# yangliu9527/Object_SLAM

Hardware: AMD Instinct MI355X
Metric: frames/sec tracking+localBA (higher is better)
Workload: dtype f64

## Files before the change

object_slam_amd/csrc/lba.hip:

```cpp
#include <hip/hip_runtime.h>
#include <string.h>
#include <type_traits>
#include <stdint.h>

#include <algorithm>
#include <atomic>
#include <chrono>
#include <condition_variable>
#include <mutex>
#include <array>
#include <vector>

#include "common.h"
#include "se3_math.h"
#include "lane_ops.h"
#include "slam_pool.h"

namespace oslam {

#ifdef OSLAM_LBA_PROFILE
#define LBA_STAMP(i) do { if (tid == 0) { long long t_ = clock64(); prof[i] += t_ - tlast; tlast = t_; } } while (0)
#else
#define LBA_STAMP(i) do { } while (0)
#endif
// ... 2035 lines not shown
        else for (int i = 0; i < 16; i++) pr.poses_out[a * 16 + i] = pr.poses[a * 16 + i];
    }
    if (gid < pr.P * 3) pr.points_out[gid] = early ? pr.points[gid] : (float)X[gid];
    if (gid == 0) { pr.stats[0] = ct->its[0]; pr.stats[1] = ct->trials[0]; pr.stats[2] = ct->its[1]; pr.stats[3] = ct->trials[1]; }
}

#include "lba_win.inc"

}

using namespace oslam;


struct oslam_lba {
    int device = 0, max_batch = 0, max_kf = 0;
    DeviceBuffer in_d, work_d, out_d;
    PinnedBuffer in_h; size_t in_off = 0;
    PinnedBuffer out_h;
    PinnedBuffer h_ctrl;
    hipStream_t strm = nullptr;
    bool owns_strm = true;
    std::mutex* launch_gate = nullptr;
    bool device_pairs = true;
    long long prof_pre_upload_ns = 0;
    int wide = 1;
    size_t win_lds_max = 0;
    int edge_rec = 1;
    int schur_vinv = 1;
    int schur_tiles = 0;
    int chol_mode = 0;
    struct Prep {
        LbaProblem pr;
        const float* p_poses = nullptr; const uint8_t* p_fixed = nullptr; const float* p_points = nullptr;
        std::vector<int> ekf, ept, pt_start, pose_start, pose_edges, pstart, chunk_kf, chunk_e0, chunk_n, kf_chunk0, pt_edge, tile_p0, tile_s0, stg_edge;
        std::vector<int> thr_own, blk_thr, blk_slots;
        int TE = 0, TP = 0, region_doubles = 0, ngroup = 1, hs_global = 0;
        std::vector<float> eobs, einfo;
        std::vector<int2> pairs;
        size_t o_poses, o_fixed, o_points, o_ekf, o_ept, o_eobs, o_einfo, o_ptstart, o_posestart, o_poseedges, o_pairs, o_pstart;
        size_t o_chunk_kf, o_chunk_e0, o_chunk_n, o_kf_chunk0, o_pt_edge, o_tile_p0, o_tile_s0, o_stg_edge, o_thr_own, o_blk_thr, o_blk_slots;
        size_t o_out_poses, o_out_points, o_out_erase, o_out_stats;
        int nfree = 0, nblk = 1; size_t npairs = 0; bool dev_pairs = false;
        int layout = 0;
        std::vector<int> order;
    };
    std::vector<Prep> prep;
    int n_prep = 0;
    PinnedBuffer h_stop;
    int* d_stop = nullptr;
    size_t lds = 0;
    hipEvent_t ev0 = nullptr, ev1 = nullptr;
    int timing = 0;
    double kern_ms = 0;
    long long kern_launches = 0;
};

static void lba_time_begin(oslam_lba* h) { if (h->timing && h->ev0) (void)hipEventRecord(h->ev0, h->strm); }
static void lba_time_end(oslam_lba* h) { if (h->timing && h->ev1) (void)hipEventRecord(h->ev1, h->strm); }
static void lba_time_collect(oslam_lba* h, long long launches) {
    if (!h->timing || !h->ev0 || !h->ev1) return;
    float ms = 0.f;
    if (hipEventElapsedTime(&ms, h->ev0, h->ev1) == hipSuccess) { h->kern_ms += ms; h->kern_launches += launches; }
}

static int arena_reserve(DeviceBuffer& q, size_t bytes) {
    if (bytes > q.cap()) OSLAM_HIP_CHECK(hipDeviceSynchronize());
    return q.grow(bytes, 1u << 20);
}

static int in_take(oslam_lba* h, size_t bytes, size_t* off) {
    const size_t need = h->in_off + ((bytes + 255) & ~(size_t)255);
    if (need > h->in_h.cap()) {
        PinnedBuffer nb;
        OSLAM_HIP_CHECK(hipStreamSynchronize(h->strm));
        OSLAM_CHECK(nb.alloc(need + need / 2 + (1u << 20)));
        if (h->in_h.ptr()) memcpy(nb.ptr(), h->in_h.ptr(), h->in_off);
        h->in_h = std::move(nb);
    }
    *off = h->in_off;
    h->in_off = need;
    return OSLAM_OK;
}
static int in_put(oslam_lba* h, const void* src, size_t bytes, size_t* off) {
    const int rc = in_take(h, bytes, off);
    if (rc) return rc;
    if (bytes) memcpy(h->in_h.bytes() + *off, src, bytes);
    return OSLAM_OK;
}

extern "C" {

int oslam_lba_kernel_time(oslam_lba_t* h, int enable, double* ms_out, long long* launches_out) {
    if (!h) { set_error("NULL handle"); return OSLAM_E_INVALID; }
    OSLAM_HIP_CHECK(hipSetDevice(h->device));
    if (enable && !h->ev0) { OSLAM_HIP_CHECK(hipEventCreate(&h->ev0)); OSLAM_HIP_CHECK(hipEventCreate(&h->ev1)); }
    if (ms_out) *ms_out = h->kern_ms;
    if (launches_out) *launches_out = h->kern_launches;
    h->kern_ms = 0; h->kern_launches = 0;
    h->timing = enable;
    return OSLAM_OK;
}

static double* s_lba_trace_buf = nullptr;
static int s_lba_trace_cap = 0;
int oslam_lba_trace(oslam_lba_t* h, int cap) {
    if (!h || cap < 0) { set_error("oslam_lba_trace: bad argument"); return OSLAM_E_INVALID; }
    OSLAM_HIP_CHECK(hipSetDevice(h->device));
    OSLAM_HIP_CHECK(hipDeviceSynchronize());
    double* none = nullptr; int zero = 0;
    OSLAM_HIP_CHECK(hipMemcpyToSymbol(HIP_SYMBOL(g_lba_trace), &none, sizeof(none)));
    OSLAM_HIP_CHECK(hipMemcpyToSymbol(HIP_SYMBOL(g_lba_trace_cap), &zero, sizeof(zero)));
    if (s_lba_trace_buf) (void)hipFree(s_lba_trace_buf);
    s_lba_trace_buf = nullptr; s_lba_trace_cap = 0;
    if (cap == 0) return OSLAM_OK;
    OSLAM_HIP_CHECK(hipMalloc((void**)&s_lba_trace_buf, sizeof(double) * (1 + 6 * (size_t)cap)));
    OSLAM_HIP_CHECK(hipMemset(s_lba_trace_buf, 0, sizeof(double) * (1 + 6 * (size_t)cap)));
    s_lba_trace_cap = cap;
    OSLAM_HIP_CHECK(hipMemcpyToSymbol(HIP_SYMBOL(g_lba_trace), &s_lba_trace_buf, sizeof(s_lba_trace_buf)));
    OSLAM_HIP_CHECK(hipMemcpyToSymbol(HIP_SYMBOL(g_lba_trace_cap), &cap, sizeof(cap)));
// ... 75 lines not shown
    memcpy(out, h->out_h.bytes() + h->prep[0].o_out_stats, 64);
    return OSLAM_OK;
}

int oslam_lba_set_mode(oslam_lba_t* h, int wide) {
    if (!h || wide < 0 || wide > 2) { set_error("oslam_lba_set_mode: mode must be 0 (compact), 1 (wide) or 2 (one workgroup per window, LDS-resident)"); return OSLAM_E_INVALID; }
    h->wide = wide;
    return OSLAM_OK;
}

int oslam_lba_set_schur(oslam_lba_t* h, int mode) {
    if (!h || mode < 0 || mode > 3) { set_error("oslam_lba_set_schur: mode must be 0 (pair gather), 1 (LDS tiles), 2 (per call) or 3 (pair gather, host-built lists)"); return OSLAM_E_INVALID; }
    h->schur_tiles = mode == 3 ? 0 : mode;
    h->device_pairs = mode != 3 && !getenv("OSLAM_LBA_HOST_PAIRS");
    return OSLAM_OK;
}

int oslam_lba_set_solver(oslam_lba_t* h, int mode) {
    if (!h || mode < 0 || mode > 4) { set_error("oslam_lba_set_solver: bad argument"); return OSLAM_E_INVALID; }
    h->chol_mode = mode;
    return OSLAM_OK;
}

volatile int32_t* oslam_lba_stop_flag(oslam_lba_t* h) { return h ? h->h_stop.as<volatile int32_t>() : nullptr; }

}

static int lba_build_tiles(oslam_lba::Prep& q, const std::vector<int>& blk, int nfree, int nP, int nE, size_t region_bytes, char* err, size_t errn) {
#pragma clang diagnostic push
#pragma clang diagnostic ignored "-Wformat-security"
    auto fail = [&](int rc, const char* fmt, auto... a) { snprintf(err, errn, fmt, a...); return rc; };
#pragma clang diagnostic pop
    const std::vector<int>& pt_start = q.pt_start;
    const std::vector<int>& ekf = q.ekf;
    const int nblk = q.nblk;
    auto tof = [&](int x, int y) { return x * nfree - x * (x - 1) / 2 + (y - x); };
    int TP = kWinTilePointsMax, TE = kWinTileEdgesMax;
    while (TE > 128 && win_tile_doubles(TE, TP) * 8 > region_bytes) TE -= 32;
    q.TE = TE; q.TP = TP;
    q.tile_p0.clear(); q.tile_s0.clear(); q.stg_edge.clear();
    std::vector<long long> load(nblk, 0);
    {
        int np = 0, ns = 0;
        q.tile_p0.push_back(0); q.tile_s0.push_back(0);
        std::vector<int> fb;
        for (int p = 0; p < nP; p++) {
            fb.clear();
            for (int i = pt_start[p]; i < pt_start[p + 1]; i++) { const int b2 = blk[ekf[q.pt_edge[i]]]; if (b2 >= 0) fb.push_back(b2); }
            const int fe = (int)fb.size();
            if (np > 0 && (np + 1 > TP || ns + fe > TE)) { q.tile_p0.push_back(p); q.tile_s0.push_back((int)q.stg_edge.size()); np = 0; ns = 0; }
            for (int i = pt_start[p]; i < pt_start[p + 1]; i++) {
                const int e = q.pt_edge[i];
                if (blk[ekf[e]] >= 0) { q.stg_edge.push_back(e); ns++; }
            }
            for (int i = 0; i < fe; i++)
                for (int j = i; j < fe; j++) load[tof(fb[i], fb[j])]++;
            np++;
        }
        q.tile_p0.push_back(nP); q.tile_s0.push_back((int)q.stg_edge.size());
    }
    q.npairs = 0;
    for (int b2 = 0; b2 < nblk; b2++) q.npairs += (size_t)load[b2];
    {
        std::vector<int> cnt(nblk, 0);
        int used = 0;
        for (int b2 = 0; b2 < nblk; b2++) if (load[b2] > 0) { cnt[b2] = 1; used++; }
        const int G = std::max(1, (used + kWinThreads - 1) / kWinThreads);
// ... 22 lines not shown
        for (size_t i = 0; i < ord.size(); i++) {
            const int b2 = ord[i].second / 64, s2 = ord[i].second % 64, g = (int)(i % G), slot = g * kWinThreads + fill[g]++;
            q.thr_own[slot] = b2 | (s2 << 16) | (cnt[b2] << 24);
            slot_of[i] = slot;
        }
        std::vector<std::vector<int>> per(nblk);
        for (size_t i = 0; i < ord.size(); i++) { const int b2 = ord[i].second / 64, s2 = ord[i].second % 64; if ((int)per[b2].size() < cnt[b2]) per[b2].resize(cnt[b2]); per[b2][s2] = slot_of[i]; }
        for (int b2 = 0; b2 < nblk; b2++) {
            q.blk_thr[b2] = (int)q.blk_slots.size() | (cnt[b2] << 16);
            for (int s2 = 0; s2 < cnt[b2]; s2++) q.blk_slots.push_back(per[b2][s2]);
        }
        if (q.blk_slots.empty()) q.blk_slots.push_back(0);
    }
    return OSLAM_OK;
}

static int lba_build(const oslam_lba_t* h, oslam_lba::Prep& q, int layout, bool want_pairs, bool use_tiles, int nKF, const float* poses, const uint8_t* fixed, int nP, const float* points,
                     int nE, const int32_t* edge_kf, const int32_t* edge_pt, const float* edge_obs, const float* edge_invSigma2, const float K5[5], int use_stop_flag,
                     const float* poses_out, const float* points_out, const uint8_t* erase, int iters0, int iters1, int nstages, int robust0, float delta_mono,
                     float delta_stereo, char* err, size_t errn) {
#pragma clang diagnostic push
#pragma clang diagnostic ignored "-Wformat-security"
    auto fail = [&](int rc, const char* fmt, auto... a) { snprintf(err, errn, fmt, a...); return rc; };
#pragma clang diagnostic pop
    if (!h || !poses || !fixed || !points || !K5 || !poses_out || !points_out || (nE > 0 && (!edge_kf || !edge_pt || !edge_obs || !edge_invSigma2 || !erase)))
        return fail(OSLAM_E_INVALID, "NULL argument");
    if (nKF < 1 || nKF > h->max_kf || nP < 0 || nE < 0)
        return fail(OSLAM_E_CAPACITY, "problem (%d keyframes, %d points, %d edges) exceeds the handle capacity (%d keyframes per window)", nKF, nP, nE, h->max_kf);
    q.layout = layout;
    q.p_poses = poses; q.p_fixed = fixed; q.p_points = points;
    std::vector<int>& pt_start = q.pt_start; std::vector<int>& pose_start = q.pose_start;
    pt_start.assign(nP + 1, 0); pose_start.assign(nKF + 1, 0);
    std::vector<int>& order = q.order;
    order.resize(nE);
    for (int i = 0; i < nE; i++) {
        if (edge_kf[i] < 0 || edge_kf[i] >= nKF || edge_pt[i] < 0 || edge_pt[i] >= nP) return fail(OSLAM_E_INVALID, "edge %d references vertex out of range", i);
        pt_start[edge_pt[i] + 1]++;
        pose_start[edge_kf[i] + 1]++;
    }
    for (int p = 0; p < nP; p++) pt_start[p + 1] += pt_start[p];
    for (int k = 0; k < nKF; k++) pose_start[k + 1] += pose_start[k];
    {
        std::vector<int> cur(pt_start.begin(), pt_start.end() - 1);
        for (int i = 0; i < nE; i++) order[cur[edge_pt[i]]++] = i;
    }
    if (layout == 1) {
        std::vector<int> cur(pose_start.begin(), pose_start.end() - 1), o2(nE);
        for (int i = 0; i < nE; i++) o2[cur[edge_kf[order[i]]]++] = order[i];
        order.swap(o2);
    }
    std::vector<int>& ekf = q.ekf; std::vector<int>& ept = q.ept;
    ekf.resize(nE); ept.resize(nE); q.eobs.resize((size_t)nE * 3); q.einfo.resize(nE);
    for (int i = 0; i < nE; i++) {
        const int sidx = order[i];
        ekf[i] = edge_kf[sidx]; ept[i] = edge_pt[sidx]; q.einfo[i] = edge_invSigma2[sidx];
        for (int k = 0; k < 3; k++) q.eobs[(size_t)i * 3 + k] = edge_obs[(size_t)sidx * 3 + k];
    }
    int nfree = 0;
    for (int k = 0; k < nKF; k++) nfree += fixed[k] ? 0 : 1;
    if (nfree > kLbaMaxKF) return fail(OSLAM_E_CAPACITY, "%d free keyframes > %d", nfree, kLbaMaxKF);
    if (h->wide == 0 && nKF > kLbaMaxKF) return fail(OSLAM_E_CAPACITY, "%d keyframes > %d (compact layout; use mode 1 or 2)", nKF, kLbaMaxKF);
    q.nfree = nfree; q.nblk = std::max(1, nfree * (nfree + 1) / 2);
    std::vector<int> blk(nKF);
    for (int k = 0, nb = 0; k < nKF; k++) blk[k] = fixed[k] ? -1 : nb++;
    auto tof = [&](int x, int y) { return x * nfree - x * (x - 1) / 2 + (y - x); };
    q.npairs = 0; q.pairs.clear(); q.pstart.clear(); q.dev_pairs = false;
    if (layout == 0) {
        q.pose_edges.resize(nE);
        std::vector<int> cur(pose_start.begin(), pose_start.end() - 1);
        for (int i = 0; i < nE; i++) q.pose_edges[cur[ekf[i]]++] = i;
        std::vector<int> seen(nKF, -1);
        for (int p = 0; p < nP; p++)
            for (int i = pt_start[p]; i < pt_start[p + 1]; i++) {
                if (seen[ekf[i]] == p) return fail(OSLAM_E_INVALID, "duplicate observation of point %d in keyframe %d", p, ekf[i]);
                seen[ekf[i]] = p;
            }
        q.tile_p0.clear();
        if (want_pairs && use_tiles) {
            q.pt_edge.resize(nE);
            for (int i = 0; i < nE; i++) q.pt_edge[i] = i;
            for (int p = 0; p < nP; p++) std::sort(q.pt_edge.begin() + pt_start[p], q.pt_edge.begin() + pt_start[p + 1], [&](int x, int y) { return ekf[x] < ekf[y]; });
            const int rc = lba_build_tiles(q, blk, nfree, nP, nE, (size_t)kWinLdsMax, err, errn);
            if (rc) return rc;
        } else if (want_pairs && h->device_pairs && h->wide == 1) {
            size_t tot = 0;
            for (int p = 0; p < nP; p++) {
                if (pt_start[p + 1] - pt_start[p] > 65534) return fail(OSLAM_E_CAPACITY, "point %d has more than 65534 observations", p);
                size_t kf_ = 0;
                for (int i = pt_start[p]; i < pt_start[p + 1]; i++) kf_ += blk[ekf[i]] >= 0;
                tot += kf_ * (kf_ + 1) / 2;
            }
            q.npairs = tot; q.dev_pairs = true;
        } else if (want_pairs) {
            const int nblk = q.nblk;
            std::vector<int>& pstart = q.pstart;
            pstart.assign(nblk + 1, 0);
            for (int p = 0; p < nP; p++)
                for (int i = pt_start[p]; i < pt_start[p + 1]; i++) {
                    const int bi = blk[ekf[i]];
                    if (bi < 0) continue;
                    for (int j = pt_start[p]; j < pt_start[p + 1]; j++) {
                        const int bj = blk[ekf[j]];
                        if (bj >= bi) pstart[tof(bi, bj) + 1]++;
// ... 14 lines not shown
                }
        }
    } else {
        q.pt_edge.resize(nE);
        {
            std::vector<int> cur(pt_start.begin(), pt_start.end() - 1);
            for (int i = 0; i < nE; i++) q.pt_edge[cur[ept[i]]++] = i;
        }
        for (int p = 0; p < nP; p++)
            for (int i = pt_start[p] + 1; i < pt_start[p + 1]; i++)
                if (ekf[q.pt_edge[i]] == ekf[q.pt_edge[i - 1]]) return fail(OSLAM_E_INVALID, "duplicate observation of point %d in keyframe %d", p, ekf[q.pt_edge[i]]);
        q.chunk_kf.clear(); q.chunk_e0.clear(); q.chunk_n.clear(); q.kf_chunk0.assign(nKF + 1, 0);
        for (int k = 0; k < nKF; k++) {
            q.kf_chunk0[k] = (int)q.chunk_kf.size();
            for (int e0 = pose_start[k]; e0 < pose_start[k + 1]; e0 += 64) { q.chunk_kf.push_back(k); q.chunk_e0.push_back(e0); q.chunk_n.push_back(std::min(64, pose_start[k + 1] - e0)); }
        }
        q.kf_chunk0[nKF] = (int)q.chunk_kf.size();
        const size_t region_bytes = h->win_lds_max - win_persist_bytes(nKF, nfree);
        size_t hs_d = (size_t)win_hs_doubles(nfree);
        q.hs_global = hs_d * 8 > region_bytes ? 1 : 0;
        if (q.hs_global) { const size_t n6 = 6 * (size_t)nfree, pw = ((n6 + 1 + kMB - 1) / kMB + 1) * kMB; hs_d = (size_t)kMB * pw + n6 + 2 * kMB; }
        { const int rc = lba_build_tiles(q, blk, nfree, nP, nE, region_bytes, err, errn); if (rc) return rc; }
        q.region_doubles = (int)std::max(hs_d, win_tile_doubles(q.TE, q.TP));
    }
    LbaProblem& pr = q.pr;
    memset(&pr, 0, sizeof(pr));
    pr.K = nKF; pr.P = nP; pr.E = nE;
    pr.stop = use_stop_flag ? h->d_stop : nullptr;
    for (int i = 0; i < 5; i++) pr.K5[i] = K5[i];
    pr.iters0 = iters0; pr.iters1 = iters1; pr.nstages = nstages; pr.robust0 = robust0; pr.delta_mono = delta_mono; pr.delta_stereo = delta_stereo;
    return OSLAM_OK;
}

static int lba_place(oslam_lba_t* h, oslam_lba::Prep& q) {
    const size_t nKF = q.pr.K, nP = q.pr.P, nE = q.pr.E;
    int rc;
    if ((rc = in_put(h, q.p_poses, nKF * 64, &q.o_poses)) || (rc = in_put(h, q.p_fixed, nKF, &q.o_fixed)) || (rc = in_put(h, q.p_points, nP * 12, &q.o_points)) ||
        (rc = in_put(h, q.ekf.data(), nE * 4, &q.o_ekf)) || (rc = in_put(h, q.ept.data(), nE * 4, &q.o_ept)) || (rc = in_put(h, q.eobs.data(), nE * 12, &q.o_eobs)) ||
        (rc = in_put(h, q.einfo.data(), nE * 4, &q.o_einfo)) || (rc = in_put(h, q.pt_start.data(), (nP + 1) * 4, &q.o_ptstart)))
        return rc;
    q.o_posestart = q.o_poseedges = q.o_pairs = q.o_pstart = q.o_chunk_kf = q.o_chunk_e0 = q.o_chunk_n = q.o_kf_chunk0 = q.o_pt_edge = 0;
    q.o_tile_p0 = q.o_tile_s0 = q.o_stg_edge = q.o_thr_own = q.o_blk_thr = q.o_blk_slots = 0;
    if (q.layout == 0) {
        if ((rc = in_put(h, q.pose_start.data(), (nKF + 1) * 4, &q.o_posestart)) || (rc = in_put(h, q.pose_edges.data(), nE * 4, &q.o_poseedges))) return rc;
        if (!q.tile_p0.empty() &&
            ((rc = in_put(h, q.tile_p0.data(), q.tile_p0.size() * 4, &q.o_tile_p0)) || (rc = in_put(h, q.tile_s0.data(), q.tile_s0.size() * 4, &q.o_tile_s0)) ||
             (rc = in_put(h, q.stg_edge.data(), q.stg_edge.size() * 4, &q.o_stg_edge)) || (rc = in_put(h, q.thr_own.data(), q.thr_own.size() * 4, &q.o_thr_own)) ||
             (rc = in_put(h, q.blk_thr.data(), q.blk_thr.size() * 4, &q.o_blk_thr)) || (rc = in_put(h, q.blk_slots.data(), q.blk_slots.size() * 4, &q.o_blk_slots))))
            return rc;
    } else {
        const size_t nc = q.chunk_kf.size();
        if ((rc = in_put(h, q.chunk_kf.data(), nc * 4, &q.o_chunk_kf)) || (rc = in_put(h, q.chunk_e0.data(), nc * 4, &q.o_chunk_e0)) || (rc = in_put(h, q.chunk_n.data(), nc * 4, &q.o_chunk_n)) ||
            (rc = in_put(h, q.kf_chunk0.data(), (nKF + 1) * 4, &q.o_kf_chunk0)) || (rc = in_put(h, q.pt_edge.data(), nE * 4, &q.o_pt_edge)) ||
            (rc = in_put(h, q.tile_p0.data(), q.tile_p0.size() * 4, &q.o_tile_p0)) || (rc = in_put(h, q.tile_s0.data(), q.tile_s0.size() * 4, &q.o_tile_s0)) ||
            (rc = in_put(h, q.stg_edge.data(), q.stg_edge.size() * 4, &q.o_stg_edge)) || (rc = in_put(h, q.thr_own.data(), q.thr_own.size() * 4, &q.o_thr_own)) ||
            (rc = in_put(h, q.blk_thr.data(), q.blk_thr.size() * 4, &q.o_blk_thr)) || (rc = in_put(h, q.blk_slots.data(), q.blk_slots.size() * 4, &q.o_blk_slots)))
            return rc;
    }
    if (q.layout == 0 && !q.pstart.empty()) {
        if ((rc = in_put(h, q.pairs.data(), q.npairs * sizeof(int2), &q.o_pairs)) || (rc = in_put(h, q.pstart.data(), q.pstart.size() * 4, &q.o_pstart))) return rc;
    }
    return OSLAM_OK;
}

constexpr int kSchurTilesMinEdges = 8000;

struct LbaArgs {
    int nKF; const float* poses; const uint8_t* fixed; int nP; const float* points; int nE; const int32_t* edge_kf; const int32_t* edge_pt; const float* edge_obs;
    const float* edge_invSigma2; float* poses_out; float* points_out; uint8_t* erase;
};

static bool win_fits(const oslam_lba_t* h, int K, int nfree) {
    if (nfree < 1 || nfree * (nfree + 1) / 2 > kWinGroupsMax * kWinThreads || nfree > kLbaMaxKF) return false;
    const size_t persist = win_persist_bytes(K, nfree);
    if (persist >= h->win_lds_max) return false;
    const size_t n6 = 6 * (size_t)nfree, pw = ((n6 + 1 + kMB - 1) / kMB + 1) * kMB;
    return persist + 8 * win_tile_doubles(128, kWinTilePointsMax) <= h->win_lds_max &&
           persist + 8 * std::min((size_t)win_hs_doubles(nfree), (size_t)kMB * pw + n6 + 2 * kMB) <= h->win_lds_max;
}

static int lba_prepare_all(oslam_lba_t* h, int n, const LbaArgs* a, const float K5[5], int use_stop_flag, int iters0, int iters1, int nstages, int robust0, float delta_mono,
                           float delta_stereo, std::vector<int>* window_rc = nullptr) {
    h->in_off = 0;
    if ((int)h->prep.size() < n) h->prep.resize(n);
    h->n_prep = n;
    std::vector<int> rcs(n, 0);
    std::vector<std::array<char, 192>> errs(n);
    long long sumE = 0;
    for (int i = 0; i < n; i++) sumE += a[i].nE;
    bool use_tiles = h->schur_tiles == 1 || (h->schur_tiles == 2 && sumE >= (long long)kSchurTilesMinEdges * n);
    std::vector<int> nfrees(n, 0);
    for (int i = 0; i < n; i++) {
        const LbaArgs& q = a[i];
        if (q.fixed && q.nKF > 0) for (int k = 0; k < q.nKF; k++) nfrees[i] += q.fixed[k] ? 0 : 1;
        if (nfrees[i] * (nfrees[i] + 1) / 2 > kWinGroupsMax * kWinThreads) use_tiles = false;
    }
    auto one = [&](int i) {
        const LbaArgs& q = a[i];
        const int nfree = nfrees[i];
        const int layout = (h->wide == 2 && win_fits(h, q.nKF, nfree)) ? 1 : 0;
        errs[i][0] = 0;
        rcs[i] = lba_build(h, h->prep[i], layout, layout == 1 || h->wide != 0, use_tiles, q.nKF, q.poses, q.fixed, q.nP, q.points, q.nE, q.edge_kf, q.edge_pt, q.edge_obs, q.edge_invSigma2, K5,
                           use_stop_flag, q.poses_out, q.points_out, q.erase, iters0, iters1, nstages, robust0, delta_mono, delta_stereo, errs[i].data(), errs[i].size());
    };
    if (n > 1) oslam_drv::shared_parallel_for(n, one);
    else one(0);
    if (window_rc) *window_rc = rcs;
    for (int i = 0; i < n; i++) if (rcs[i]) { set_error("%s", errs[i].data()); return rcs[i]; }
    if (window_rc) window_rc->assign(n, 0);
    for (int i = 0; i < n; i++) { const int rc = lba_place(h, h->prep[i]); if (rc) return rc; }
    return OSLAM_OK;
}

static int lba_launch(oslam_lba_t* h) {
    const auto t_launch0 = std::chrono::steady_clock::now();
    const int n = h->n_prep;
    OSLAM_HIP_CHECK(hipSetDevice(h->device));
    hipStream_t st = h->strm;
    int rc;
    std::vector<int> idx0, idx1;
    for (int i = 0; i < n; i++) (h->prep[i].layout == 1 ? idx1 : idx0).push_back(i);
    const int n0 = (int)idx0.size(), n1 = (int)idx1.size();
    const bool wide = h->wide != 0;
    size_t o_probs, o_ws, o_wins, o_order;
    if ((rc = in_take(h, sizeof(LbaProblem) * n, &o_probs)) || (rc = in_take(h, sizeof(LbaWide) * std::max(n0, 1), &o_ws)) || (rc = in_take(h, sizeof(LbaWin) * std::max(n1, 1), &o_wins)) ||
        (rc = in_take(h, sizeof(int) * std::max(n1, 1), &o_order)))
        return rc;
    size_t work = 0, outb = 0;
    auto takeW = [&](size_t bytes) { const size_t at = work; work += (bytes + 255) & ~(size_t)255; return at; };
    auto takeO = [&](size_t bytes) { const size_t at = outb; outb += (bytes + 255) & ~(size_t)255; return at; };
    struct WOff { size_t Xa, Xb, chi2, level, Hpl, Hll, Dinv, bl, xl, Hpp, bp, Hs, xp, ctrl, T, R, blk, free_pose, partF, partS, partM, W, rec, eoi, chunkC, pairPart, parts, pairM, pairsW, pstartW; };
    bool tiles = wide && n0 > 0;
    for (int i : idx0) tiles = tiles && !h->prep[i].tile_p0.empty();
    const bool use_rec = wide && !tiles && h->schur_vinv && h->edge_rec;
    const int nwg_call = std::max(1, std::min(16, (2 * 256 + std::max(n0, 1) - 1) / std::max(n0, 1)));
    size_t tiles_lds = 0, packed_lds = 0, ldsm_lds = 0;
    int maxWg = 1, maxSum = 1, min_n6_big = 1 << 30;
    std::vector<WOff> wo(n);
    bool any_dev_pairs = false;
    int maxNbPt = 1, maxK = 1, maxE = 1, maxBlk = 1, maxFin = 1, maxInit = 1, max_slots = 0, min_group = 4, max_n6 = 0;
    bool all_lds = true;
    const size_t ctrl_base = takeW(sizeof(LbaCtrl) * std::max(n0, 1));
    size_t win_lds = 0;
// ... 203 lines not shown
                    else { if (use_rec) OSLAM_UPD_LANES(true, false); else OSLAM_UPD_LANES(false, false); }
#undef OSLAM_UPD_LANES
#undef OSLAM_UPD_LAUNCH
                    if (!fold_ctrl) hipLaunchKernelGGL(k_w_ctrlB, dim3(1, n0), dim3(256), 0, st, d_probs, d_ws);
                }
            }
            OSLAM_HIP_CHECK(copy_to_host_async(h->h_ctrl.as<LbaCtrl>(), Wk + ctrl_base, sizeof(LbaCtrl) * n0, st));
            OSLAM_HIP_CHECK(stream_wait(st));
            bool all_done = true;
            int n_active = 0;
            for (int i = 0; i < n0; i++) { all_done = all_done && h->h_ctrl.as<LbaCtrl>()[i].done != 0; n_active += h->h_ctrl.as<LbaCtrl>()[i].done == 0; }
            if (call_stats) fprintf(stderr, "[lba call] %d windows, %d slots done, %d active\n", n0, slots_done, n_active);
            if (all_done) break;
            if (handle_gate.owns_lock() && gate_release_frac > 0 && (double)n_active <= gate_release_frac * n0) handle_gate.unlock();
            group = 4;
        }
        hipLaunchKernelGGL(k_w_final, dim3(div_up(maxFin, 256), n0), dim3(256), 0, st, d_probs, d_ws);
        const int n_chol = (chol_ldsm ? 1 : 0) + (chol_packed ? 1 : 0) + (chol_mfma ? 1 : 0);
        launches += 3 + (1 + (tiles ? 3 : 2) + std::max(n_chol, 1) + (fold_ctrl ? 1 : 2)) * (long long)slots_done;
    }
    lba_time_end(h);
    OSLAM_HIP_CHECK(hipGetLastError());
    OSLAM_HIP_CHECK(copy_to_host_async(h->out_h.bytes(), O, outb, st));
    OSLAM_HIP_CHECK(stream_wait(st));
    lba_time_collect(h, launches);
    return OSLAM_OK;
}

static void lba_fetch(oslam_lba_t* h, int i, float* poses_out, float* points_out, uint8_t* erase, int32_t* stats) {
    const oslam_lba::Prep& q = h->prep[i];
    memcpy(poses_out, h->out_h.bytes() + q.o_out_poses, (size_t)q.pr.K * 64);
    if (q.pr.P > 0) memcpy(points_out, h->out_h.bytes() + q.o_out_points, (size_t)q.pr.P * 12);
    const uint8_t* er = h->out_h.bytes() + q.o_out_erase;
    for (int e = 0; e < q.pr.E; e++) erase[q.order[e]] = er[e];
    if (stats) { const int* st = (const int*)(h->out_h.bytes() + q.o_out_stats); for (int k = 0; k < 4; k++) stats[k] = st[k]; }
}

extern "C" {

int oslam_lba_optimize(oslam_lba_t* h, int nKF, const float* poses, const uint8_t* fixed, int nP, const float* points, int nE,
                       const int32_t* edge_kf, const int32_t* edge_pt, const float* edge_obs, const float* edge_invSigma2,
                       const float K5[5], int use_stop_flag, float* poses_out, float* points_out, uint8_t* erase, int32_t stats[4]) {
    if (!h) { set_error("NULL handle"); return OSLAM_E_INVALID; }
    const LbaArgs a = {nKF, poses, fixed, nP, points, nE, edge_kf, edge_pt, edge_obs, edge_invSigma2, poses_out, points_out, erase};
    int rc = lba_prepare_all(h, 1, &a, K5, use_stop_flag, 5, 10, 2, 1, (float)sqrt(5.991), (float)sqrt(7.815));
    if (!rc) rc = lba_launch(h);
    if (!rc) lba_fetch(h, 0, poses_out, points_out, erase, stats);
    return rc;
}

int oslam_ba_optimize(oslam_lba_t* h, int nKF, const float* poses, const uint8_t* fixed, int nP, const float* points, int nE,
                      const int32_t* edge_kf, const int32_t* edge_pt, const float* edge_obs, const float* edge_invSigma2,
                      const float K5[5], int nIterations, int bRobust, int use_stop_flag, float* poses_out, float* points_out) {
    if (!h) { set_error("NULL handle"); return OSLAM_E_INVALID; }
    if (nIterations < 0) { set_error("nIterations < 0"); return OSLAM_E_INVALID; }
    std::vector<uint8_t> erase(nE > 0 ? nE : 1);
    const LbaArgs a = {nKF, poses, fixed, nP, points, nE, edge_kf, edge_pt, edge_obs, edge_invSigma2, poses_out, points_out, erase.data()};
    int rc = lba_prepare_all(h, 1, &a, K5, use_stop_flag, nIterations, 0, 1, bRobust ? 1 : 0, (float)sqrt(5.99), (float)sqrt(7.815));
    if (!rc) rc = lba_launch(h);
    if (!rc) lba_fetch(h, 0, poses_out, points_out, erase.data(), nullptr);
    return rc;
}

int oslam_lba_optimize_batch(oslam_lba_t* h, int n, const oslam_lba_problem_t* probs, const float K5[5]) {
    if (!h || !probs || !K5) { set_error("NULL argument"); return OSLAM_E_INVALID; }
    if (n < 1 || n > h->max_batch) { set_error("batch %d outside [1,%d]", n, h->max_batch); return OSLAM_E_INVALID; }
    std::vector<LbaArgs> a(n);
// ... 59 lines not shown
```

object_slam_amd/csrc/slam_driver.hip:

```cpp
#include <atomic>
#include <chrono>
#include <map>
#include <memory>

#include "common.h"
#include "slam_map.h"
#include "slam_pool.h"

int oslam_slam_make_hip_ops(const oslam_slam_config_t* cfg, oslam_slam_ops_t* out);

namespace oslam_drv {

struct Vocab {
    uint64_t top[10][4], sub[10][10][4];
    Vocab() {
        uint64_t s = 0x853c49e6748fea9bULL;
        auto next = [&]() {
            const uint64_t old = s;
            s = old * 6364136223846793005ULL + 1442695040888963407ULL;
            const uint32_t x = (uint32_t)(((old >> 18u) ^ old) >> 27u), r = (uint32_t)(old >> 59u);
            return (x >> r) | (x << ((-r) & 31));
        };
        auto word = [&]() { const uint64_t hi = next(); const uint64_t lo = next(); return (hi << 32) | lo; };
        for (int i = 0; i < 10; i++)
// ... 146 lines not shown
        std::fill(counter.begin(), counter.end(), 0);
        std::fill(mpMark.begin(), mpMark.end(), 0ull);
        std::fill(baMark.begin(), baMark.end(), 0);
        std::fill(fuseMark.begin(), fuseMark.end(), 0);
        voteVersion = -1; votePts.clear();
        mapVersion++; locVersion = -1; locWalkFrame = -1; locKFs.clear(); locListPending = false;
        resetRequested = false;
    }
    std::vector<int> updList;
    std::vector<std::unique_ptr<BowViews>> kfBow;
    BowViews& bow_views(const Ctx& c, int kf);
};

struct Ctx {
    oslam_slam_config_t cfg;
    oslam_slam_ops_t ops;
    int S = 0, cap = 0;
    float scale[OSLAM_MAX_LEVELS], invScale[OSLAM_MAX_LEVELS], sigma2[OSLAM_MAX_LEVELS], invSigma2[OSLAM_MAX_LEVELS];
    float bounds[4];
    float invfx, invfy, thDepth, mb, logScale;
    int maxFrames, minFrames;
    bool stereo = false;
    Vocab voc;
    const oslam_voc_t* realVoc = nullptr;
    bool started = false;
    double bowSec = 0; long long bowKFs = 0, bowDesc = 0;
    std::vector<std::unique_ptr<Seq>> seq;
    std::unique_ptr<Pool> pool;
    double sec[16] = {0};
    double cpu[16] = {0};
    double fine[8] = {0};
    CpuAccount acct;
    int shard = 0;
    struct Win {
        int si = -1, nLocal = 0, nFree = 0;
        std::vector<int> kfs, pts; std::vector<float> poses, points, eobs, einv, poses_out, points_out; std::vector<uint8_t> fixed, erase;
        std::vector<int32_t> ekf, ept; std::vector<std::pair<int, int>> eref;
        std::vector<int32_t> pstart, uref; std::vector<uint8_t> eoct, pquirk, uskip; std::vector<float> ulsf, uOw, uout5;
        int32_t st[4] = {0, 0, 0, 0};
        void reset() { kfs.clear(); pts.clear(); poses.clear(); points.clear(); eobs.clear(); einv.clear(); poses_out.clear(); points_out.clear(); fixed.clear(); erase.clear(); ekf.clear(); ept.clear(); eref.clear(); nLocal = 0; }
    };
    std::vector<Win> winPool;
    struct PendingLM { bool active = false, submitted = false; std::vector<int> who; std::vector<Win*> wins; std::vector<oslam_lba_problem_t> probs; } pend;
    std::unique_ptr<MpUpdate> updTrack, updMap;
    int mapStep = 0;
    std::vector<Map::JrScratch> jrScratch;
    int injectLbaFailure = -1;
    bool residentPts = false;
    std::atomic<long long> badKFObs{0};
    std::atomic<long long> contentCounter{0}, locReuse{0}, locFrames{0};
    long long next_content_id() { return contentCounter.fetch_add(1, std::memory_order_relaxed) + 1; }
    int mask_stride = 0, masks_on_device = 0;
};

}

using namespace oslam_drv;

struct oslam_slam { Ctx c; };

namespace oslam_drv {

static void compute_bow(const Ctx& c, int N, const uint8_t* desc, std::vector<uint32_t>& out) {
    if (!out.empty()) return;
    out.resize(N);
    if (c.realVoc) {
        (void)oslam_voc_transform_host(c.realVoc, desc, N, 4, nullptr, out.data(), nullptr);
        return;
    }
    for (int i = 0; i < N; i++) out[i] = c.voc.node(desc + (size_t)i * 32);
// ... 1364 lines not shown
                    if (i + kPF < n) { const int pq = kp_[i + kPF]; if (pq >= 0 && bam[pq] != cur) __builtin_prefetch(&m.mps[pq].obs); }
                    const int p = kp_[i];
                    if (p < 0 || bam[p] == cur) continue;
                    bam[p] = cur;

                    if (!m.pBad[p]) { W.pts.push_back(p); edgeCap += m.mps[p].obs.size(); }
                }
            }
            std::vector<int>& slot = s.counter;
            for (int q = 0; q < W.nLocal; q++) slot[W.kfs[q]] = q + 1;
            W.points.resize(W.pts.size() * 3);
            W.ekf.resize(edgeCap); W.ept.resize(edgeCap); W.eobs.resize(edgeCap * 3); W.einv.resize(edgeCap); W.eref.resize(edgeCap); W.eoct.resize(edgeCap);
            W.pstart.resize(W.pts.size() + 1); W.pquirk.assign(W.pts.size(), 0);
            size_t ne = 0;
            for (size_t j = 0; j < W.pts.size(); j++) {
                prefetch_okp_ahead(m.mps, W.pts, j, W.pts.size());
                const int p = W.pts[j];
                const MapPt& mp = m.mps[p];
                W.pstart[j] = (int32_t)ne;
                for (int d = 0; d < 3; d++) W.points[j * 3 + d] = mp.pos[d];
                for (size_t oi = 0; oi < mp.obs.size(); oi++) {
                    const int kid = mp.obs[oi].first;
                    int q = slot[kid];
                    if (q == 0) {
                        if (m.kfs[kid].bad) { W.pquirk[j] = 1; continue; }
                        W.kfs.push_back(kid);
                        slot[kid] = q = (int)W.kfs.size();
                    }
                    const ObsKp& kp = mp.okp[oi];
                    W.ekf[ne] = q - 1; W.ept[ne] = (int)j;
                    W.eobs[ne * 3] = kp.x; W.eobs[ne * 3 + 1] = kp.y; W.eobs[ne * 3 + 2] = kp.ur;
                    W.einv[ne] = c.invSigma2[kp.octave];
                    W.eoct[ne] = (uint8_t)kp.octave;
                    W.eref[ne] = std::make_pair(kid, p);
                    ne++;
                }
            }
            W.pstart[W.pts.size()] = (int32_t)ne;
            W.ekf.resize(ne); W.ept.resize(ne); W.eobs.resize(ne * 3); W.einv.resize(ne); W.eref.resize(ne); W.eoct.resize(ne);
            int nFreeCap = W.nLocal;
            {
                int nFreeKF = 0;
                for (int q = 0; q < W.nLocal; q++) {
                    nFreeKF += W.kfs[q] != 0;
                    if (nFreeKF > kLbaMaxFreeKFs) { nFreeCap = q; break; }
                }
                if (nFreeCap < W.nLocal) s.lbaWindowsDegraded++;
            }
            W.nFree = nFreeCap;
            W.poses.resize(W.kfs.size() * 16); W.fixed.resize(W.kfs.size());
            for (size_t q = 0; q < W.kfs.size(); q++) {
                memcpy(&W.poses[q * 16], m.kfs[W.kfs[q]].pose.Tcw.m, 64);
                W.fixed[q] = (int)q >= nFreeCap ? 1 : (W.kfs[q] == 0 ? 2 : 0);
            }
            for (size_t q = 0; q < W.kfs.size(); q++) slot[W.kfs[q]] = 0;
            W.poses_out.resize(W.poses.size()); W.points_out.resize(W.points.size() + 3); W.erase.assign(W.ekf.size() + 1, 0);
            s.st[5]++; s.st[14] += (int64_t)W.ekf.size();
            s.lbaWin[0] += W.nLocal; s.lbaWin[1] += (int64_t)W.kfs.size() - W.nLocal; s.lbaWin[2] += (int64_t)W.pts.size(); s.lbaWin[3] += (int64_t)W.ekf.size();
        });
        std::vector<Win*> wins;
        for (int w = 0; w < nW; w++) if (pool_w[w].si >= 0) wins.push_back(&pool_w[w]);
        std::vector<oslam_lba_problem_t> probs(wins.size());
        for (size_t i = 0; i < wins.size(); i++) {
            Win& W = *wins[i];
            oslam_lba_problem_t& p = probs[i];
            p.nKF = (int)W.kfs.size(); p.poses = W.poses.data(); p.fixed = W.fixed.data(); p.nP = (int)W.pts.size(); p.points = W.points.data();
            p.nE = (int)W.ekf.size(); p.edge_kf = W.ekf.data(); p.edge_pt = W.ept.data(); p.edge_obs = W.eobs.data(); p.edge_invSigma2 = W.einv.data();
// ... 943 lines not shown
```

Measured before the change: 47550.

## Skip host edge reorder when already point-major and parallelize staging fill

When input edges are already sorted by point and layout 0 is used, the host-side reordering and copying of edge arrays is skipped, and caller arrays are used directly. Staging into the pinned buffer is split into a serial offset reservation pass and a parallel copy pass across windows, with pose_edges built directly in the pinned buffer. The erase scatter becomes a memcpy in the identity case, and the driver's edge vectors use a no-init allocator so resize does not zero-fill. This is aimed at CPU preparation overhead per localBA call, at the cost of more code paths and reliance on caller arrays staying alive until they are copied.

```diff
diff --git a/object_slam_amd/csrc/lba.hip b/object_slam_amd/csrc/lba.hip
--- a/object_slam_amd/csrc/lba.hip
+++ b/object_slam_amd/csrc/lba.hip
@@ -2091,7 +2091,7 @@
     struct Prep {
         LbaProblem pr;
         const float* p_poses = nullptr; const uint8_t* p_fixed = nullptr; const float* p_points = nullptr;
-        std::vector<int> ekf, ept, pt_start, pose_start, pose_edges, pstart, chunk_kf, chunk_e0, chunk_n, kf_chunk0, pt_edge, tile_p0, tile_s0, stg_edge;
+        std::vector<int> ekf, ept, pt_start, pose_start, pose_cur, pstart, chunk_kf, chunk_e0, chunk_n, kf_chunk0, pt_edge, tile_p0, tile_s0, stg_edge;
         std::vector<int> thr_own, blk_thr, blk_slots;
         int TE = 0, TP = 0, region_doubles = 0, ngroup = 1, hs_global = 0;
         std::vector<float> eobs, einfo;
@@ -2102,6 +2102,8 @@
         int nfree = 0, nblk = 1; size_t npairs = 0; bool dev_pairs = false;
         int layout = 0;
         std::vector<int> order;
+        bool identity = false;
+        const int* s_ekf = nullptr; const int* s_ept = nullptr; const float* s_eobs = nullptr; const float* s_einfo = nullptr;
     };
     std::vector<Prep> prep;
     int n_prep = 0;
@@ -2138,12 +2140,6 @@
     }
     *off = h->in_off;
     h->in_off = need;
-    return OSLAM_OK;
-}
-static int in_put(oslam_lba* h, const void* src, size_t bytes, size_t* off) {
-    const int rc = in_take(h, bytes, off);
-    if (rc) return rc;
-    if (bytes) memcpy(h->in_h.bytes() + *off, src, bytes);
     return OSLAM_OK;
 }
 
@@ -2285,7 +2281,7 @@
     auto fail = [&](int rc, const char* fmt, auto... a) { snprintf(err, errn, fmt, a...); return rc; };
 #pragma clang diagnostic pop
     const std::vector<int>& pt_start = q.pt_start;
-    const std::vector<int>& ekf = q.ekf;
+    const int* ekf = q.s_ekf;
     const int nblk = q.nblk;
     auto tof = [&](int x, int y) { return x * nfree - x * (x - 1) / 2 + (y - x); };
     int TP = kWinTilePointsMax, TE = kWinTileEdgesMax;
@@ -2374,30 +2370,40 @@
     std::vector<int>& pt_start = q.pt_start; std::vector<int>& pose_start = q.pose_start;
     pt_start.assign(nP + 1, 0); pose_start.assign(nKF + 1, 0);
     std::vector<int>& order = q.order;
-    order.resize(nE);
-    for (int i = 0; i < nE; i++) {
+    bool point_major = true;
+    for (int i = 0, last = 0; i < nE; i++) {
         if (edge_kf[i] < 0 || edge_kf[i] >= nKF || edge_pt[i] < 0 || edge_pt[i] >= nP) return fail(OSLAM_E_INVALID, "edge %d references vertex out of range", i);
         pt_start[edge_pt[i] + 1]++;
         pose_start[edge_kf[i] + 1]++;
+        point_major = point_major && edge_pt[i] >= last;
+        last = edge_pt[i];
     }
     for (int p = 0; p < nP; p++) pt_start[p + 1] += pt_start[p];
     for (int k = 0; k < nKF; k++) pose_start[k + 1] += pose_start[k];
-    {
-        std::vector<int> cur(pt_start.begin(), pt_start.end() - 1);
-        for (int i = 0; i < nE; i++) order[cur[edge_pt[i]]++] = i;
-    }
-    if (layout == 1) {
-        std::vector<int> cur(pose_start.begin(), pose_start.end() - 1), o2(nE);
-        for (int i = 0; i < nE; i++) o2[cur[edge_kf[order[i]]]++] = order[i];
-        order.swap(o2);
-    }
-    std::vector<int>& ekf = q.ekf; std::vector<int>& ept = q.ept;
-    ekf.resize(nE); ept.resize(nE); q.eobs.resize((size_t)nE * 3); q.einfo.resize(nE);
-    for (int i = 0; i < nE; i++) {
-        const int sidx = order[i];
-        ekf[i] = edge_kf[sidx]; ept[i] = edge_pt[sidx]; q.einfo[i] = edge_invSigma2[sidx];
-        for (int k = 0; k < 3; k++) q.eobs[(size_t)i * 3 + k] = edge_obs[(size_t)sidx * 3 + k];
-    }
+    q.identity = point_major && layout == 0;
+    if (q.identity) {
+        order.clear();
+        q.s_ekf = edge_kf; q.s_ept = edge_pt; q.s_eobs = edge_obs; q.s_einfo = edge_invSigma2;
+    } else {
+        order.resize(nE);
+        {
+            std::vector<int> cur(pt_start.begin(), pt_start.end() - 1);
+            for (int i = 0; i < nE; i++) order[cur[edge_pt[i]]++] = i;
+        }
+        if (layout == 1) {
+            std::vector<int> cur(pose_start.begin(), pose_start.end() - 1), o2(nE);
+            for (int i = 0; i < nE; i++) o2[cur[edge_kf[order[i]]]++] = order[i];
+            order.swap(o2);
+        }
+        q.ekf.resize(nE); q.ept.resize(nE); q.eobs.resize((size_t)nE * 3); q.einfo.resize(nE);
+        for (int i = 0; i < nE; i++) {
+            const int sidx = order[i];
+            q.ekf[i] = edge_kf[sidx]; q.ept[i] = edge_pt[sidx]; q.einfo[i] = edge_invSigma2[sidx];
+            for (int k = 0; k < 3; k++) q.eobs[(size_t)i * 3 + k] = edge_obs[(size_t)sidx * 3 + k];
+        }
+        q.s_ekf = q.ekf.data(); q.s_ept = q.ept.data(); q.s_eobs = q.eobs.data(); q.s_einfo = q.einfo.data();
+    }
+    const int* ekf = q.s_ekf; const int* ept = q.s_ept;
     int nfree = 0;
     for (int k = 0; k < nKF; k++) nfree += fixed[k] ? 0 : 1;
     if (nfree > kLbaMaxKF) return fail(OSLAM_E_CAPACITY, "%d free keyframes > %d", nfree, kLbaMaxKF);
@@ -2408,9 +2414,6 @@
     auto tof = [&](int x, int y) { return x * nfree - x * (x - 1) / 2 + (y - x); };
     q.npairs = 0; q.pairs.clear(); q.pstart.clear(); q.dev_pairs = false;
     if (layout == 0) {
-        q.pose_edges.resize(nE);
-        std::vector<int> cur(pose_start.begin(), pose_start.end() - 1);
-        for (int i = 0; i < nE; i++) q.pose_edges[cur[ekf[i]]++] = i;
         std::vector<int> seen(nKF, -1);
         for (int p = 0; p < nP; p++)
             for (int i = pt_start[p]; i < pt_start[p + 1]; i++) {
@@ -2491,17 +2494,31 @@
     return OSLAM_OK;
 }
 
-static int lba_place(oslam_lba_t* h, oslam_lba::Prep& q) {
+static int lba_place(oslam_lba_t* h, oslam_lba::Prep& q, bool copy) {
     const size_t nKF = q.pr.K, nP = q.pr.P, nE = q.pr.E;
+    auto in_put = [copy](oslam_lba_t* h_, const void* src, size_t bytes, size_t* off) {
+        if (!copy) return in_take(h_, bytes, off);
+        if (bytes) memcpy(h_->in_h.bytes() + *off, src, bytes);
+        return (int)OSLAM_OK;
+    };
     int rc;
     if ((rc = in_put(h, q.p_poses, nKF * 64, &q.o_poses)) || (rc = in_put(h, q.p_fixed, nKF, &q.o_fixed)) || (rc = in_put(h, q.p_points, nP * 12, &q.o_points)) ||
-        (rc = in_put(h, q.ekf.data(), nE * 4, &q.o_ekf)) || (rc = in_put(h, q.ept.data(), nE * 4, &q.o_ept)) || (rc = in_put(h, q.eobs.data(), nE * 12, &q.o_eobs)) ||
-        (rc = in_put(h, q.einfo.data(), nE * 4, &q.o_einfo)) || (rc = in_put(h, q.pt_start.data(), (nP + 1) * 4, &q.o_ptstart)))
+        (rc = in_put(h, q.s_ekf, nE * 4, &q.o_ekf)) || (rc = in_put(h, q.s_ept, nE * 4, &q.o_ept)) || (rc = in_put(h, q.s_eobs, nE * 12, &q.o_eobs)) ||
+        (rc = in_put(h, q.s_einfo, nE * 4, &q.o_einfo)) || (rc = in_put(h, q.pt_start.data(), (nP + 1) * 4, &q.o_ptstart)))
         return rc;
-    q.o_posestart = q.o_poseedges = q.o_pairs = q.o_pstart = q.o_chunk_kf = q.o_chunk_e0 = q.o_chunk_n = q.o_kf_chunk0 = q.o_pt_edge = 0;
-    q.o_tile_p0 = q.o_tile_s0 = q.o_stg_edge = q.o_thr_own = q.o_blk_thr = q.o_blk_slots = 0;
+    if (!copy) {
+        q.o_posestart = q.o_poseedges = q.o_pairs = q.o_pstart = q.o_chunk_kf = q.o_chunk_e0 = q.o_chunk_n = q.o_kf_chunk0 = q.o_pt_edge = 0;
+        q.o_tile_p0 = q.o_tile_s0 = q.o_stg_edge = q.o_thr_own = q.o_blk_thr = q.o_blk_slots = 0;
+    }
     if (q.layout == 0) {
-        if ((rc = in_put(h, q.pose_start.data(), (nKF + 1) * 4, &q.o_posestart)) || (rc = in_put(h, q.pose_edges.data(), nE * 4, &q.o_poseedges))) return rc;
+        if ((rc = in_put(h, q.pose_start.data(), (nKF + 1) * 4, &q.o_posestart))) return rc;
+        if (!copy) { if ((rc = in_take(h, nE * 4, &q.o_poseedges))) return rc; }
+        else {
+            int* pose_edges = (int*)(h->in_h.bytes() + q.o_poseedges);
+            std::vector<int>& cur = q.pose_cur;
+            cur.assign(q.pose_start.begin(), q.pose_start.end() - 1);
+            for (int i = 0; i < (int)nE; i++) pose_edges[cur[q.s_ekf[i]]++] = i;
+        }
         if (!q.tile_p0.empty() &&
             ((rc = in_put(h, q.tile_p0.data(), q.tile_p0.size() * 4, &q.o_tile_p0)) || (rc = in_put(h, q.tile_s0.data(), q.tile_s0.size() * 4, &q.o_tile_s0)) ||
              (rc = in_put(h, q.stg_edge.data(), q.stg_edge.size() * 4, &q.o_stg_edge)) || (rc = in_put(h, q.thr_own.data(), q.thr_own.size() * 4, &q.o_thr_own)) ||
@@ -2567,7 +2584,10 @@
     if (window_rc) *window_rc = rcs;
     for (int i = 0; i < n; i++) if (rcs[i]) { set_error("%s", errs[i].data()); return rcs[i]; }
     if (window_rc) window_rc->assign(n, 0);
-    for (int i = 0; i < n; i++) { const int rc = lba_place(h, h->prep[i]); if (rc) return rc; }
+    for (int i = 0; i < n; i++) { const int rc = lba_place(h, h->prep[i], false); if (rc) return rc; }
+    auto fill = [&](int i) { (void)lba_place(h, h->prep[i], true); };
+    if (n > 1) oslam_drv::shared_parallel_for(n, fill);
+    else fill(0);
     return OSLAM_OK;
 }
 
@@ -2837,7 +2857,8 @@
     memcpy(poses_out, h->out_h.bytes() + q.o_out_poses, (size_t)q.pr.K * 64);
     if (q.pr.P > 0) memcpy(points_out, h->out_h.bytes() + q.o_out_points, (size_t)q.pr.P * 12);
     const uint8_t* er = h->out_h.bytes() + q.o_out_erase;
-    for (int e = 0; e < q.pr.E; e++) erase[q.order[e]] = er[e];
+    if (q.identity) { if (q.pr.E > 0) memcpy(erase, er, (size_t)q.pr.E); }
+    else for (int e = 0; e < q.pr.E; e++) erase[q.order[e]] = er[e];
     if (stats) { const int* st = (const int*)(h->out_h.bytes() + q.o_out_stats); for (int k = 0; k < 4; k++) stats[k] = st[k]; }
 }
 
diff --git a/object_slam_amd/csrc/slam_driver.hip b/object_slam_amd/csrc/slam_driver.hip
--- a/object_slam_amd/csrc/slam_driver.hip
+++ b/object_slam_amd/csrc/slam_driver.hip
@@ -202,10 +202,16 @@
     double fine[8] = {0};
     CpuAccount acct;
     int shard = 0;
+    template <class T> struct NoInitAlloc : std::allocator<T> {
+        template <class U> struct rebind { typedef NoInitAlloc<U> other; };
+        template <class U> void construct(U* p) { ::new ((void*)p) U; }
+        template <class U, class... A> void construct(U* p, A&&... a) { ::new ((void*)p) U(std::forward<A>(a)...); }
+    };
+    struct EdgeRef { int first, second; };
     struct Win {
         int si = -1, nLocal = 0, nFree = 0;
-        std::vector<int> kfs, pts; std::vector<float> poses, points, eobs, einv, poses_out, points_out; std::vector<uint8_t> fixed, erase;
-        std::vector<int32_t> ekf, ept; std::vector<std::pair<int, int>> eref;
+        std::vector<int> kfs, pts; std::vector<float> poses, points, poses_out, points_out; std::vector<uint8_t> fixed, erase;
+        std::vector<float, NoInitAlloc<float>> eobs, einv; std::vector<int32_t, NoInitAlloc<int32_t>> ekf, ept; std::vector<EdgeRef, NoInitAlloc<EdgeRef>> eref;
         std::vector<int32_t> pstart, uref; std::vector<uint8_t> eoct, pquirk, uskip; std::vector<float> ulsf, uOw, uout5;
         int32_t st[4] = {0, 0, 0, 0};
         void reset() { kfs.clear(); pts.clear(); poses.clear(); points.clear(); eobs.clear(); einv.clear(); poses_out.clear(); points_out.clear(); fixed.clear(); erase.clear(); ekf.clear(); ept.clear(); eref.clear(); nLocal = 0; }
@@ -1636,7 +1642,7 @@
                     W.eobs[ne * 3] = kp.x; W.eobs[ne * 3 + 1] = kp.y; W.eobs[ne * 3 + 2] = kp.ur;
                     W.einv[ne] = c.invSigma2[kp.octave];
                     W.eoct[ne] = (uint8_t)kp.octave;
-                    W.eref[ne] = std::make_pair(kid, p);
+                    W.eref[ne] = Ctx::EdgeRef{kid, p};
                     ne++;
                 }
             }
```

After: 47480. No clear change (-0.1%).
